# yashnaray/VQ-VAE-HMM-model

Hardware: AMD Instinct MI355X
Metric: VAE_HMM train-step sequences/sec (K=3, T=200, D=5) at 1/2/4/8 MI355X (higher is better)
Workload: dtype f32; 1 GPU; cfg2: VAE_HMM train step (compute_loss+backward+Adam); global_batch=1024, per_gpu_batch=1024, seq_len=200, K=3, input_dim=5, hidden_dim=64, hidden_dim2=32, u_dim=4, trans_hidden=128, parallelism=single, hip_graph=False, step_form=fused (Adam in the backward's tail launch), eager

## Files before the change

### vq-vae-hmm-model_amd/csrc/api.hip

```cpp
#include "vqhmm.h"

#include <math.h>
#include <stdio.h>
#include <stdlib.h>
#include <string.h>

#include <algorithm>

#include "kernels.h"


using namespace vqhmm;

namespace {

enum P {
  ENC1_W, ENC1_B, ENC2_W, ENC2_B, LOGIT_W, LOGIT_B, LOG_PRIOR, TN0_W, TN0_B, TN2_W, TN2_B,
  EMB, DEC1_W, DEC1_B, DEC2_W, DEC2_B, PAR_W, PAR_B
};

struct Carver {
  char* base;
  size_t off = 0;
  template <class T>
// ... 1247 lines not shown
      break;
    }
    case S_REDUCE: nm = p.wgroup && tail_fused_on() ? "tail" : "grad_tail"; break;
    case S_COMPOSE_BWD: nm = p.wgroup ? (tail_fused_on() ? "tail" : "adam") : "compose_bwd"; break;
    case S_LOGPRIOR: nm = p.wgroup && tail_fused_on() ? "tail" : "grad_tail"; break;
  }
  snprintf(out, len, "%s", nm);
  return VQHMM_OK;
}

int vqhmm_elbo_stage_f32(const vqhmm_dims_t* d, const float* const* w, const float* x, const float* u, int u_layout,
                         const int64_t* lengths, const int64_t* norm, int64_t B, int64_t T, float beta, void* ws,
                         size_t ws_bytes, float* grad, int stage, void* stream) {
  if (!dims_ok(d) || !w || !ws || stage < 0 || stage >= S_COUNT) return VQHMM_EINVAL;
  ElboPlan p = plan_elbo(d, B, T, ws);
  if (ws_bytes < p.bytes) return VQHMM_EWORKSPACE;
  StepCtx c{w, x, u, u_layout, lengths, norm, beta, 1, p.loss, nullptr, nullptr, grad, nullptr};
  return run_stage(p, c, stage, (hipStream_t)stream);
}

int vqhmm_elbo_pieces(const vqhmm_dims_t* d, int64_t B, int64_t T, const void* ws, const float** loss,
                      const float** pieces) {
  if (!dims_ok(d) || !ws) return VQHMM_EINVAL;
  ElboPlan p = plan_elbo(d, B, T, const_cast<void*>(ws));
  if (loss) *loss = p.loss;
  if (pieces) *pieces = p.pieces;
  return VQHMM_OK;
}

int vqhmm_elbo_status_offset(const vqhmm_dims_t* d, int64_t B, int64_t T, size_t* offset) {
  if (!dims_ok(d) || B <= 0 || T <= 0 || !offset) return VQHMM_EINVAL;
  char* const base = reinterpret_cast<char*>(4096);
  const ElboPlan p = plan_elbo(d, B, T, base);
  *offset = (size_t)(reinterpret_cast<char*>(p.sync + 2) - base);
  return VQHMM_OK;
}

int vqhmm_elbo_debug_buffers(const vqhmm_dims_t* d, int64_t B, int64_t T, const void* ws, const float** out) {
  if (!dims_ok(d) || !ws || !out) return VQHMM_EINVAL;
  ElboPlan p = plan_elbo(d, B, T, const_cast<void*>(ws));
  const float* v[16] = {p.xp, p.h1e, p.h2e, p.logits, p.q, p.g1, p.g2, p.par,
                        p.dpar, p.dg2, p.dg1, p.dqd, p.dlog, p.dh2, p.dh1, p.dqx};
  for (int i = 0; i < 16; ++i) out[i] = v[i];
  return VQHMM_OK;
}

int vqhmm_debug_prof(int which, uint64_t* out, int64_t n) {
  if (!out || n < 0 || n > 256 * 16) return VQHMM_EINVAL;
  switch (which) {
    case 0: return strip_prof_copy(out, n);
    case 1: return conv2_prof_copy(out, n);
    case 2: return head_prof_copy(out, n);
    case 3: return bwdw_prof_copy(out, n);
  }
  return VQHMM_EINVAL;
}

int vqhmm_adam_f32(float* param, const float* grad, float* exp_avg, float* exp_avg_sq, int64_t n, double lr,
                   double beta1, double beta2, double eps, int64_t* step, float grad_scale, void* stream) {
  if (n < 0 || !step || (n > 0 && (!param || !grad || !exp_avg || !exp_avg_sq))) return VQHMM_EINVAL;
  return launch_adam(param, grad, exp_avg, exp_avg_sq, n, lr, beta1, beta2, eps, step, grad_scale,
                     (hipStream_t)stream);
}

int vqhmm_clip_grad_norm_f32(float* grad, int64_t n, float pre_scale, float max_norm, float* total_norm,
                              void* stream) {
  if (n < 0 || (n > 0 && !grad) || !(max_norm > 0.f)) return VQHMM_EINVAL;
  return launch_clip_grad_norm(grad, n, pre_scale, max_norm, total_norm, (hipStream_t)stream);
}

int vqhmm_gather_chunks_f32(const float* src, const int64_t* meta, int64_t B, int64_t C, int64_t Tmax, float* out,
                            void* stream) {
  if (B < 0 || C < 0 || Tmax < 0 || C > INT32_MAX || Tmax > INT32_MAX) return VQHMM_EINVAL;
  if (B * C * Tmax > 0 && (!src || !meta || !out)) return VQHMM_EINVAL;
  return launch_gather_chunks(src, meta, B, C, Tmax, out, (hipStream_t)stream);
}

int vqhmm_infer_workspace_size(const vqhmm_dims_t* d, int64_t B, int64_t T, size_t* bytes) {
  if (!dims_ok(d) || B < 0 || T < 0 || !bytes) return VQHMM_EINVAL;
  const int64_t R = B * (T + 2);
  const int hw = ld4(d->hidden_dim > d->hidden_dim2 ? d->hidden_dim : d->hidden_dim2);
  Carver c{nullptr};
  c.take<float>(R * hw);
  c.take<float>(R * hw);
  c.take<float>(R * ld4(d->K));
  c.take<float>(R * ld4(d->input_dim > d->K ? d->input_dim : d->K));
  c.take<float>((size_t)d->hidden_dim * d->K * 3);
  *bytes = c.off + 256;
  return VQHMM_OK;
}

static int encode_impl(const vqhmm_dims_t* d, const float* const* w, const float* x, int64_t B, int64_t T,
                       float* logits_cf, float* q_cf, float* q_pcl, float* xin, float* bufA, float* bufB,
                       hipStream_t s, int32_t* regimes = nullptr) {
  const int64_t R = B * (T + 2);
  int rc;
  if ((rc = launch_to_pcl(x, d->input_dim, B, (int)T, T, 1, xin, s))) return rc;
  ConvArgs a{};
  a.R = R; a.T = (int)T;
  a.src = xin; a.Kc = d->input_dim; a.ks = 3; a.W = w[ENC1_W]; a.bias = w[ENC1_B];
  a.N = d->hidden_dim; a.act = 1; a.out = bufA;
  if ((rc = launch_conv(a, s))) return rc;
  a = ConvArgs{};
  a.R = R; a.T = (int)T;
  a.src = bufA; a.Kc = d->hidden_dim; a.ks = 3; a.W = w[ENC2_W]; a.bias = w[ENC2_B]; a.N = d->hidden_dim2;
  a.act = 1; a.out = bufB;
// ... 428 lines not shown
```

### vq-vae-hmm-model_amd/csrc/kernels.h

```cpp
#pragma once
#include "common.h"

namespace vqhmm {

struct ConvArgs {
  const float* src;
  int src_cf;
  int Kc;
  int64_t R;
  int T;
  int ks;
  const float* W;
  int w_dgrad;
  const float* Wimg;
  const float* bias;
  const float* scale;
  int N;
  int act;
  const float* aux;
  float* out;
  float* out_cf;
  const float* tW;
  const float* tb;
  int C2;
// ... 154 lines not shown
int launch_conv(const ConvArgs& a, hipStream_t s);
enum ConvKind { CONV_UNSUPPORTED, CONV_CONV2, CONV_BIG, CONV_BIG_TAIL, CONV_MM, CONV_MM_TAIL, CONV_MM_TAIL_SPLIT };
struct ConvChoice {
  int kind;
  int cfg;
  size_t lds;
};
ConvChoice conv_choice(const ConvArgs& a);
void conv_family(const ConvArgs& a, char* out, size_t n);
bool convbig_supported(const ConvArgs& a);
int launch_convbig(const ConvArgs& a, hipStream_t s);
bool conv2_supported(const ConvArgs& a);
bool conv2_fused_supported(const ConvArgs& a);
int launch_conv2_fused(const ConvArgs& a, hipStream_t s);
bool conv2_bwd_pair_supported(const ConvArgs& a, const ConvArgs& f);
int launch_conv2_bwd_pair(const ConvArgs& a, const ConvArgs& f, hipStream_t s);
struct WImgJob {
  const float* W;
  const float* E;
  int composed, H;
  int w_dgrad, N, Kc, ks;
  float* img;
};
__host__ __device__ inline int c2_nb(int N) { return N <= 16 ? 1 : N <= 32 ? 2 : 4; }
__host__ __device__ inline int c2_kcp(int Kc) { return Kc <= 16 ? 1 : Kc <= 32 ? 2 : 4; }
__host__ __device__ inline int c2_ldx(int Kc) { return 16 * c2_kcp(Kc) + 8; }
__host__ __device__ inline int64_t c2_image_floats(int N, int Kc, int ks) {
  return (int64_t)ks * 16 * c2_nb(N) * c2_ldx(Kc);
}
int launch_conv2(const ConvArgs& a, hipStream_t s);
bool strip_fwd_supported(const ConvArgs& e1, const ConvArgs& e2, const ConvArgs& d1, const ConvArgs& d2);
bool strip_head_supported(const HeadArgs& h);
int strip_fwd_grid(int64_t R);
int launch_strip_fwd(const ConvArgs& e1, const ConvArgs& e2, const ConvArgs& d1, const ConvArgs& d2, const HeadArgs* h,
                     hipStream_t s);
bool strip_bwd_supported(const ConvArgs& pd, const ConvArgs& d2, const ConvArgs& f, const ConvArgs& e2);
int launch_strip_bwd(const ConvArgs& pd, const ConvArgs& d2, const ConvArgs& f, const ConvArgs& e2, hipStream_t s);
struct StripWgradArgs {
  const float* x;
  const float* cmpW;
  float* slab[6];
  float* bslab[6];
  float* cslab;
  int D, K, H2;
  int64_t* step_inc;
  int store;
};
bool strip_bwdw_supported(const ConvArgs& pd, const ConvArgs& d2, const ConvArgs& f, const ConvArgs& e2, int D);
int strip_bwdw_own(int64_t R);
int strip_bwdw_grid(int64_t R);
int launch_strip_bwdw(const ConvArgs& pd, const ConvArgs& d2, const ConvArgs& f, const ConvArgs& e2,
                      const StripWgradArgs& w, hipStream_t s);
int strip_prof_copy(uint64_t* out, int64_t n);
int conv2_prof_copy(uint64_t* out, int64_t n);
int head_prof_copy(uint64_t* out, int64_t n);
int bwdw_prof_copy(uint64_t* out, int64_t n);
int launch_wgrad(const WgradArgs& a, hipStream_t s);
enum WgradKind { WGRAD_UNSUPPORTED, WGRAD_2, WGRAD_BIG, WGRAD_GENERIC };
int wgrad_choice(const WgradArgs& a);
const char* wgrad_family(const WgradArgs& a);
bool wgradbig_supported(const WgradArgs& a);
int64_t wgradbig_rows(int64_t R, int N, int C);
int launch_wgradbig(const WgradArgs& a, hipStream_t s);
int64_t wgrad_chunks(int64_t R, int64_t tiles);
bool wgrad2_supported(const WgradArgs& a);
int64_t wgrad2_rows(int64_t R, int N, int C, int ks);
int launch_wgrad2(const WgradArgs& a, hipStream_t s);
constexpr int MAX_WJOBS = 8;
struct WgradGroup {
  WgradArgs job[MAX_WJOBS];
  int variant[MAX_WJOBS], wn[MAX_WJOBS], wc[MAX_WJOBS];
  int64_t blk0[MAX_WJOBS + 1];
  int njobs;
  int64_t* step_inc;
};
bool wgrad2_group_supported(const WgradArgs& a);
int64_t wgrad2_group_rows(int64_t rows, int N, int C, int ks);
int launch_wgrad2_group(const WgradArgs* jobs, int n, hipStream_t s, int64_t* step_inc = nullptr);
struct StagedHeadArgs {
  int64_t B;
  int T;
  int64_t R;
  int D, K;
  const float *x, *par, *logits, *q;
  const int64_t* lengths;
  const float* log_prior;
  float* log_pi;
  float* lgA;
  float *nx, *dqc, *trw;
  float beta;
  const int64_t* norm;
  int need_grad;
  float *dpar, *dlx, *dqx;
  double* part;
  float* q0;
};
bool staged_head_supported(int K);
bool fused_head_supported(const HeadArgs& a);
enum FusedHeadKind { HEAD_NONE, HEAD_MFMA, HEAD_SCALAR };
int fused_head_kind(const HeadArgs& a);
enum StagedL1 { L1_NONE, L1_LANES16, L1_POW2_32, L1_POW2_16, L1_WIDE4, L1_WIDE, L1_LANES64 };
int staged_l1_variant(int K);
const char* staged_l1_name(int K);
int launch_staged_head(const StagedHeadArgs& a, int l2grid, hipStream_t s);

int head_grid(int64_t R);
// ... 145 lines not shown
```

### vq-vae-hmm-model_amd/csrc/strip.hip

```cpp
#include "vqhmm.h"

#include <stddef.h>
#include <stdlib.h>

#include "prof.h"
#include "strip_dev.h"

namespace vqhmm {

struct StripFwdArgs {
  int64_t R;
  int T, D, H2, K, P;
  const float* xp;
  const float *img_e1, *img_d1;
  const float *img_e2, *img_d2;
  const float *b_e1, *b_e2, *b_d1, *b_d2;
  const float *tWl, *tbl;
  const float *tWp, *tbp;
  float *h1e, *h2e, *logits, *q, *g1, *g2, *par;
  int64_t nstrip;
  int dbg;
};

namespace {

template <int NB2>
struct StripFwdLds {
  static constexpr int NW2 = 16 * NB2;
  float We2[3 * NW2 * ST_LDW];
  float Wd2[3 * 64 * ST_LDW];
  float Ee2[NW2 * 17 + 16];
  float Ed2[64 * 17 + 16];
  float Wf[2][3 * 64 * 8];
  float bf[2][64];
  float Xx[ST_XR * ST_XLD];
  float Xq[ST_XR * ST_XLD];
  float slot[8][18 * ST_LDW];
  unsigned long long hcnt[8];
};

template <int TH>
struct StripHeadW {
  static constexpr int LDW2 = TH + 4;
  float W2S[16 * LDW2];
  float W1S[TH * 8];
};
struct StripHeadLds {
  static constexpr int LDL = 20;
  float uS[ST_WIN * 8];
  float lgS[ST_WIN * LDL];
  float dlgS[ST_WIN * LDL];
  float aS[ST_WIN * 4];
  float wS[ST_WIN];
  double red[8][4];
  float q0w[8][4];
};

__device__ __forceinline__ void pk_weights(const float* Wf, int C, int lg4, int l16, float (&w)[4][4]) {
#pragma unroll
  for (int e = 0; e < 4; ++e) {
    const int k = 4 * lg4 + e;
    const bool in = k < 3 * C;
    const int tap = in ? k / C : 0, c = in ? k - tap * C : 0;
#pragma unroll
    for (int nb = 0; nb < 4; ++nb) {
      const float v = Wf[(tap * 64 + nb * 16 + l16) * 8 + c];
      w[nb][e] = in ? v : 0.f;
    }
  }
}

__device__ __forceinline__ void pk_block(const float (&w)[4][4], const float* Xw, int C, int lg4, int l16,
                                         f32x4 (&acc)[4]) {
  float b[4];
#pragma unroll
  for (int e = 0; e < 4; ++e) {
    const int k = 4 * lg4 + e;
    const bool in = k < 3 * C;
    const int tap = in ? k / C : 0, c = in ? k - tap * C : 0;
    const float v = Xw[(l16 + tap) * ST_XLD + c];
    b[e] = in ? v : 0.f;
  }
#pragma unroll
  for (int nb = 0; nb < 4; ++nb) {
    acc[nb] = f32x4{0.f, 0.f, 0.f, 0.f};
#pragma unroll
    for (int e = 0; e < 4; ++e) acc[nb] = mfma16x16x4(w[nb][e], b[e], acc[nb]);
  }
}

__device__ __forceinline__ void front_epi(f32x4 (&acc)[4], const f32x4 (&bias)[4], int64_t r0, int64_t R, int T,
                                          int lg4, int l16, int slo, int shi, float* out, float* xs,
                                          bool nostore, int only = -1, float* xlo = nullptr,
                                          float* xhi = nullptr) {
  const int64_t r = r0 + l16;
  const bool valid = row_valid(r, R, T);
  const bool st = l16 >= slo && l16 < shi && r < R && !nostore;
#pragma unroll
  for (int nb = 0; nb < 4; ++nb) {
    f32x4 y;
#pragma unroll
    for (int v = 0; v < 4; ++v) {
      const float yy = relu_f(acc[nb][v] * 1.0f + bias[nb][v]);
      y[v] = valid ? yy : 0.f;
    }
    acc[nb] = y;
    if (st) *reinterpret_cast<f32x4*>(out + r * 64 + nb * 16 + 4 * lg4) = y;
    if (only < 0 || l16 == only) *reinterpret_cast<f32x4*>(xs + l16 * ST_LDW + nb * 16 + 4 * lg4) = y;
    if (xlo && l16 == 0) *reinterpret_cast<f32x4*>(xlo + nb * 16 + 4 * lg4) = y;
    if (xhi && l16 == 15) *reinterpret_cast<f32x4*>(xhi + nb * 16 + 4 * lg4) = y;
  }
}

template <int NB>
struct TailConsts {
  f32x4 bias[NB], tw[NB], tb;
  __device__ __forceinline__ void load(const float* Es, int lg4, int l16) {
    constexpr int NW = 16 * NB;
#pragma unroll
    for (int nb = 0; nb < NB; ++nb) {
      const float4 b4 = *reinterpret_cast<const float4*>(Es + nb * 16 + 4 * lg4);
      const float4 t4 = *reinterpret_cast<const float4*>(Es + NW + l16 * NW + nb * 16 + 4 * lg4);
      bias[nb] = f32x4{b4.x, b4.y, b4.z, b4.w};
      tw[nb] = f32x4{t4.x, t4.y, t4.z, t4.w};
    }
    const float4 t4 = *reinterpret_cast<const float4*>(Es + 17 * NW + 4 * lg4);
    tb = f32x4{t4.x, t4.y, t4.z, t4.w};
  }
};

template <int NB, bool SM>
__device__ __forceinline__ void tail_epi(f32x4 (&acc)[NB], const TailConsts<NB>& k, int64_t r0, int64_t R, int T,
                                         int lg4, int l16, int slo, int shi, int N, float* out, int C2, float* t_out,
                                         float* q_out, float* xq, bool nostore) {
  const int64_t r = r0 + l16;
  const bool valid = row_valid(r, R, T);
  const bool st = l16 >= slo && l16 < shi && r < R && !nostore;
  const int ldn = ld4(N), ldt = ld4(C2);
#pragma unroll
  for (int nb = 0; nb < NB; ++nb) {
    f32x4 y;
#pragma unroll
    for (int v = 0; v < 4; ++v) {
      const float yy = relu_f(acc[nb][v] * 1.0f + k.bias[nb][v]);
      y[v] = valid ? yy : 0.f;
    }
    acc[nb] = y;
    const int n0 = nb * 16 + 4 * lg4;
    if (st && n0 < ldn) *reinterpret_cast<f32x4*>(out + r * ldn + n0) = y;
  }
  f32x4 z = k.tb;
#pragma unroll
  for (int nb = 0; nb < NB; ++nb)
#pragma unroll
    for (int v = 0; v < 4; ++v) z = mfma16x16x4(k.tw[nb][v], acc[nb][v], z);
  const int c0 = 4 * lg4;
#pragma unroll
  for (int v = 0; v < 4; ++v) z[v] = valid ? z[v] : 0.f;
  if (st && c0 < ldt) *reinterpret_cast<f32x4*>(t_out + r * ldt + c0) = z;
  if constexpr (SM) {
    float m = -__builtin_inff();
#pragma unroll
    for (int v = 0; v < 4; ++v)
      if (c0 + v < C2) m = fmaxf(m, z[v]);
    m = fmaxf(m, xor16(m));
    m = fmaxf(m, xor32(m));
    float e[4], s = 0.f;
#pragma unroll
    for (int v = 0; v < 4; ++v) {
      e[v] = (c0 + v < C2) ? __expf(z[v] - m) : 0.f;
      s += e[v];
    }
    s += xor16(s);
    s += xor32(s);
    f32x4 qv;
#pragma unroll
    for (int v = 0; v < 4; ++v) qv[v] = valid ? e[v] / s : 0.f;
    if (st && c0 < ldt) *reinterpret_cast<f32x4*>(q_out + r * ldt + c0) = qv;
    if (c0 == 0) {
      *reinterpret_cast<f32x4*>(xq + l16 * ST_XLD) = qv;
      *reinterpret_cast<f32x4*>(xq + l16 * ST_XLD + 4) = z;
    }
  }
}

template <int NW>
__device__ __forceinline__ const float* es_src(const float* bias, int N, const float* tW, const float* tb, int C2, int i,
                                               bool& ok) {
  const bool in_b = i < NW, in_w = !in_b && i < 17 * NW;
  const int j = in_w ? i - NW : 0, c2w = j / NW, n = j - c2w * NW, c2b = (!in_b && !in_w) ? i - 17 * NW : 0;
// ... 43 lines not shown

  auto load_x = [&](int64_t s0) {
    const int row = tid >> 1, h = 4 * (tid & 1);
    int64_t r = s0 - 2 + row;
    r = r < 0 ? 0 : (r >= R ? R - 1 : r);
    return *reinterpret_cast<const float4*>(a.xp + r * ldx + (h < ldx ? h : 0));
  };
  auto store_x = [&](int64_t s0, float4 v) {
    if (tid < 2 * ST_XR) {
      const int row = tid >> 1, h = 4 * (tid & 1);
      const int64_t r = s0 - 2 + row;
      const bool ok = r >= 0 && r < R && h < ldx;
      *reinterpret_cast<float4*>(sh.Xx + row * ST_XLD + h) = ok ? v : make_float4(0.f, 0.f, 0.f, 0.f);
    }
  };

  constexpr int HKP = 4, HB = HTH > 0 ? HTH / 16 : 1, HLDW2 = HTH + 4, HNW = HTH > 0 ? 16 * HLDW2 + HTH * 8 : 1;
  constexpr int HNJ = (HNW + 511) / 512;
  const int prow = tid >> 2, si = tid & 3;
  float hwv[HNJ];
  if constexpr (HTH > 0) {
    const int KK = h.K * h.K;
#pragma unroll
    for (int j = 0; j < HNJ; ++j) {
      const int i = tid + 512 * j;
      float v = 0.f;
      if (i < 16 * HLDW2) {
        const int ij = i / HLDW2, hh = i - ij * HLDW2;
        v = (ij < KK && hh < HTH) ? h.W2[ij * HTH + hh] : 0.f;
      } else if (i < HNW) {
        const int k = i - 16 * HLDW2, hh = k >> 3, c = k & 7;
        v = c < h.U ? h.W1[hh * h.U + c] : (c == h.U ? h.b1[hh] : 0.f);
      }
      hwv[j] = v;
    }
    if (!h.norm && !h.cnt_in) {
      unsigned long long c = 0;
      for (int64_t b = tid; b < h.B; b += 512) {
        const int64_t L = h.lengths[b];
        c += (unsigned long long)(L <= 0 ? 0 : (L < T ? L : T));
      }
#pragma unroll
      for (int o = 32; o >= 1; o >>= 1) c += __shfl_xor(c, o);
      if (lane == 0) sh.hcnt[wave] = c;
    }
  }
  stamp<PROF>(0);
  if constexpr (PROF > 0) { if (threadIdx.x == 0 && blockIdx.x < 256) g_prof[blockIdx.x * 16 + 13] = __builtin_amdgcn_s_memtime(); }
  for (int j = wave; wave < 4 && j < 12; j += 4) {
    const int g = j * 64 + lane, img = g / 384, i = g - img * 384, row = i >> 1, h = 4 * (i & 1);
    dma16((img ? a.img_d1 : a.img_e1) + row * ST_LDF + h, &sh.Wf[0][0] + j * 256);
  }
  int64_t s = blockIdx.x;
  float4 px = load_x(s * ST_OWN - ST_HALO);
  constexpr int NE = NW2 * 17 + 16, ND = 64 * 17 + 16, NC = NE + ND + 128;
  constexpr int NCJ = (NC + 511) / 512;
  float cv[NCJ];
  bool cvok[NCJ];
#pragma unroll
  for (int j = 0; j < NCJ; ++j) {
    const int i = tid + 512 * j;
    bool oke, okd;
    const float* pe = es_src<NW2>(a.b_e2, a.H2, a.tWl, a.tbl, a.K, i < NE ? i : 0, oke);
    const float* pd = es_src<64>(a.b_d2, 64, a.tWp, a.tbp, a.P, (i >= NE && i < NE + ND) ? i - NE : 0, okd);
    const int ib = (i >= NE + ND && i < NC) ? i - NE - ND : 0;
    const bool inE = i < NE, inD = !inE && i < NE + ND, inB = !inE && !inD && i < NC;
    const bool ok = inE ? oke : inD ? okd : inB;
    const float* p = inE ? pe : inD ? pd : (ib < 64 ? a.b_e1 : a.b_d1) + (ib & 63);
    cv[j] = *(ok ? p : a.b_e1);
    cvok[j] = ok;
  }
#pragma unroll
  for (int j = 0; j < NCJ; ++j) cv[j] = cvok[j] ? cv[j] : 0.f;
  {
    constexpr int N1 = 3 * NW2 * ST_LDW / 4, N2 = 3 * 64 * ST_LDW / 4;
    constexpr int C1 = (N1 + 63) / 64, C2 = (N2 + 63) / 64;
    constexpr int NJ = (C1 + C2 + 7) / 8;
#pragma unroll
    for (int jj = 0; jj < NJ; ++jj) {
      const int c = min(wave + 8 * jj, C1 + C2 - 1);
      const bool first = c < C1;
      const int cc = first ? c : c - C1;
      const int i = cc * 64 + lane;
      if (i < (first ? N1 : N2)) dma16((first ? a.img_e2 : a.img_d2) + 4 * i, (first ? sh.We2 : sh.Wd2) + cc * 256);
    }
  }
  static_assert(offsetof(S, Ed2) == offsetof(S, Ee2) + NE * 4, "constant blocks must be contiguous");
#pragma unroll
  for (int j = 0; j < NCJ; ++j) {
    const int i = tid + 512 * j;
    if (i < NE + ND) sh.Ee2[i] = cv[j];
    else if (i < NC) sh.bf[0][i - NE - ND] = cv[j];
  }
  if (tid < 4 * ST_XLD) sh.Xq[(tid < 2 * ST_XLD ? 0 : (ST_XR - 4) * ST_XLD) + tid] = 0.f;
  store_x(s * ST_OWN - ST_HALO, px);
  lds_barrier();
  stamp<PROF>(1);
  float wE[4][4], wD[4][4];
  pk_weights(sh.Wf[0], a.D, lg4, l16, wE);
  pk_weights(sh.Wf[1], a.K, lg4, l16, wD);
  f32x4 bE[4], bD[4];
#pragma unroll
  for (int nb = 0; nb < 4; ++nb) {
    const float4 e4 = *reinterpret_cast<const float4*>(sh.bf[0] + nb * 16 + 4 * lg4);
    const float4 d4 = *reinterpret_cast<const float4*>(sh.bf[1] + nb * 16 + 4 * lg4);
    bE[nb] = f32x4{e4.x, e4.y, e4.z, e4.w};
    bD[nb] = f32x4{d4.x, d4.y, d4.z, d4.w};
  }
  TailConsts<NB2> kE;
  TailConsts<4> kD;
  if constexpr (HTH == 0) {
    kE.load(sh.Ee2, lg4, l16);
    kD.load(sh.Ed2, lg4, l16);
  }
  static_assert(HTH == 0 || (offsetof(S, Xx) == offsetof(S, bf) + 2 * 64 * 4 &&
                             sizeof(StripHeadW<HTH>) <= offsetof(S, Xx) - offsetof(S, Wf) &&
                             sizeof(StripHeadLds) <= sizeof(float) * 8 * 18 * ST_LDW),
                "the head's LDS fits the regions it reuses");
  float lp_i = 0.f, inv_n = 1.f, cpri = 0.f, cent = 0.f;
  const bool hgrad = h.need_grad != 0;
  if constexpr (HTH > 0) {
    unsigned long long cnt;
    if (h.norm) cnt = (unsigned long long)h.norm[0];
    else if (h.cnt_in) cnt = (unsigned long long)*h.cnt_in;
    else cnt = ((((((sh.hcnt[0] + sh.hcnt[1]) + sh.hcnt[2]) + sh.hcnt[3]) + sh.hcnt[4]) + sh.hcnt[5]) + sh.hcnt[6]) + sh.hcnt[7];
    inv_n = 1.0f / fmaxf((float)(cnt * (unsigned long long)h.D), 1.0f);
    const float Bn = loss_norm_batch(h.norm, h.B);
    cpri = -h.beta / Bn;
    cent = h.beta / Bn;
    float m = -__builtin_inff();
    for (int k = 0; k < h.K; ++k) m = fmaxf(m, h.log_prior[k]);
    float se = 0.f;
    for (int k = 0; k < h.K; ++k) se += __expf(h.log_prior[k] - m);
    if (si < h.K) lp_i = h.log_prior[si] - (m + __logf(se));
  }
  float s_rec = 0.f, s_ent = 0.f, s_tr = 0.f, s_init = 0.f, q0acc = 0.f, db2acc = 0.f;
  f32x4 gW2 = f32x4{0.f, 0.f, 0.f, 0.f}, gW1 = gW2;

  const int mlo = ST_HALO - 16 * wave, mhi = ST_HALO + ST_OWN - 16 * wave;
  const int slo = max(0, mlo), shi = min(16, mhi);
  const bool nost = a.dbg & 1;
  int it = 0;
  for (; s < a.nstrip; s += gridDim.x) {
    const int64_t s0 = s * ST_OWN - ST_HALO;
    const int64_t rb = s0 + 16 * wave;
    {
      const int64_t nx = s + gridDim.x;
      px = load_x((nx < a.nstrip ? nx : s) * ST_OWN - ST_HALO);
    }
    {
      f32x4 acc[4];
      pk_block(wE, sh.Xx + (16 * wave + 1) * ST_XLD, a.D, lg4, l16, acc);
      front_epi(acc, bE, rb, R, T, lg4, l16, slo, shi, a.h1e, slot + ST_LDW, nost, -1,
                wave > 0 ? sh.slot[wave - 1] + 17 * ST_LDW : nullptr, wave < 7 ? sh.slot[wave + 1] : nullptr);
      if (wave == 5 || wave == 6) {
        const bool lo = wave == 5;
        f32x4 acc2[4];
        pk_block(wE, sh.Xx + (lo ? 0 : 16 * 7 + 2) * ST_XLD, a.D, lg4, l16, acc2);
        front_epi(acc2, bE, lo ? s0 - 1 : s0 + 16 * 7 + 1, R, T, lg4, l16, 0, 0, a.h1e,
                  lo ? sh.slot[0] : sh.slot[7] + 2 * ST_LDW, true, lo ? 0 : 15);
      }
    }
    if (it == 0) asm volatile("s_waitcnt vmcnt(0)" ::: "memory");
    lds_barrier();
    {
      f32x4 acc[NB2][1];
#pragma unroll
      for (int nb = 0; nb < NB2; ++nb) acc[nb][0] = f32x4{0.f, 0.f, 0.f, 0.f};
      c2_mfma_tile<NB2, 1, 4, 3, ST_LDW, NW2>(sh.We2, slot, lg4, l16, acc, true);
      f32x4 y[NB2];
#pragma unroll
      for (int nb = 0; nb < NB2; ++nb) y[nb] = acc[nb][0];
      if constexpr (HTH > 0) kE.load(sh.Ee2, lg4, l16);
      tail_epi<NB2, true>(y, kE, rb, R, T, lg4, l16, slo, shi, a.H2, a.h2e, a.K, a.logits, a.q,
                          sh.Xq + (16 * wave + 2) * ST_XLD, nost);
    }
    lds_barrier();
    if (it == 0) stamp<PROF>(2);
    if constexpr (HTH > 0) {
      if (it == 0) {
        float* hw = &sh.Wf[0][0];
#pragma unroll
        for (int j = 0; j < HNJ; ++j)
          if (tid + 512 * j < HNW) hw[tid + 512 * j] = hwv[j];
      }
    }
    {
      f32x4 acc[4];
      pk_block(wD, sh.Xq + (16 * wave + 1) * ST_XLD, a.K, lg4, l16, acc);
      if constexpr (PROF > 0) {
        if (it == 0) {
          asm volatile("s_nop 0" : : "v"(acc[3][3]));
          stamp<PROF>(10);
        }
      }
      front_epi(acc, bD, rb, R, T, lg4, l16, slo, shi, a.g1, slot + ST_LDW, nost, -1,
                wave > 0 ? sh.slot[wave - 1] + 17 * ST_LDW : nullptr, wave < 7 ? sh.slot[wave + 1] : nullptr);
      if (it == 0) stamp<PROF>(11);
    }
    lds_barrier();
    if (it == 0) stamp<PROF>(4);
    {
      f32x4 acc[4][1];
#pragma unroll
      for (int nb = 0; nb < 4; ++nb) acc[nb][0] = f32x4{0.f, 0.f, 0.f, 0.f};
      c2_mfma_tile<4, 1, 4, 3, ST_LDW, 64>(sh.Wd2, slot, lg4, l16, acc, true);
      f32x4 y[4];
#pragma unroll
      for (int nb = 0; nb < 4; ++nb) y[nb] = acc[nb][0];
      if constexpr (PROF > 0) {
        if (it == 0) {
          asm volatile("s_nop 0" : : "v"(y[3][3]));
          stamp<PROF>(5);
        }
      }
      if constexpr (HTH > 0) kD.load(sh.Ed2, lg4, l16);
      tail_epi<4, false>(y, kD, rb, R, T, lg4, l16, slo, shi, 64, a.g2, a.P, a.par, nullptr, nullptr, nost);
    }
    if (it == 0) stamp<PROF>(6);
    {
      const int64_t nx = s + gridDim.x;
      store_x((nx < a.nstrip ? nx : s) * ST_OWN - ST_HALO, px);
    }
    if constexpr (HTH > 0) __syncthreads();
    else lds_barrier();
    if (it == 0) stamp<PROF>(3);
    if constexpr (HTH > 0) {
      StripHeadLds& hs = *reinterpret_cast<StripHeadLds*>(&sh.slot[0][0]);
      const StripHeadW<HTH>& hw = *reinterpret_cast<const StripHeadW<HTH>*>(&sh.Wf[0][0]);
      constexpr int LDL = StripHeadLds::LDL;
      const int K = h.K, U = h.U, D = h.D, KK = K * K;
      const int ldp = ld4(2 * D), ldxh = ld4(D), ldu = ld4(U);
      const int64_t r = s0 + ST_HALO + prow;
      const unsigned Tp = (unsigned)T + 2u;
      const unsigned rcl = (unsigned)(r < R ? r : R - 1);
      const int b = (int)(rcl / Tp);
      const int t = (int)(rcl - (unsigned)b * Tp) - 1;
      const bool valid = r < R && prow <= ST_OWN && t >= 0 && t < T;
      const bool own = prow < ST_OWN && r < R;
      const int64_t L = h.lengths[b];
      const bool m = valid && t < L;
      const float wgt = (valid && t >= 1 && t < L) ? 1.f : 0.f;
      const float* qrow = sh.Xq + (ST_HALO + prow + 2) * ST_XLD;
      float qv[HKP];
#pragma unroll
      for (int k = 0; k < HKP; ++k) qv[k] = (valid && k < K) ? qrow[k] : 0.f;
      const float qp = (valid && t >= 1 && si < K) ? qrow[si - ST_XLD] : 0.f;
      float qi = 0.f;
#pragma unroll
      for (int k = 0; k < HKP; ++k) qi = si == k ? qv[k] : qi;
      float mu[2], lv[2], xv[2];
#pragma unroll
      for (int k = 0; k < 2; ++k) {
        const int c = min(si + HKP * k, D - 1);
        mu[k] = h.par[(int64_t)rcl * ldp + c];
        lv[k] = h.par[(int64_t)rcl * ldp + D + c];
        xv[k] = h.x[(int64_t)rcl * ldxh + c];
      }
      const float uu = h.u[(int64_t)rcl * ldu + min(si, ldu - 1)];
#pragma unroll
      for (int c = si; c < 8; c += HKP) hs.uS[prow * 8 + c] = c < U ? (valid ? uu : 0.f) : (c == U ? 1.f : 0.f);
      for (int i = tid; i < ST_WIN * LDL; i += 512)
        if (i % LDL >= KK) hs.dlgS[i] = 0.f;
      lds_barrier();
      {
        f32x4 lg;
#pragma unroll
        for (int v = 0; v < 4; ++v) {
          const int ij = 4 * lg4 + v;
          lg[v] = ij < KK ? h.b2[ij] : 0.f;
        }
        const float ub = hs.uS[(wave * 16 + l16) * 8 + lg4];
#pragma unroll 2
        for (int hb = 0; hb < HB; ++hb) {
          const float w1a = lg4 < U ? hw.W1S[(hb * 16 + l16) * 8 + lg4] : 0.f;
          f32x4 bb;
#pragma unroll
          for (int v = 0; v < 4; ++v) bb[v] = hw.W1S[(hb * 16 + 4 * lg4 + v) * 8 + U];
// ... 330 lines not shown
      for (int nb = 0; nb < 4; ++nb) y[nb] = acc[nb][0];
      mask_epi(y, m2, 1.0f, rb, R, T, lg4, l16, slo, shi, a.dh1, nullptr, 0);
    }
    ++it;
  }
  if constexpr (PROF > 0) {
    __syncthreads();
    stamp<PROF>(7);
    if (threadIdx.x == 0 && blockIdx.x < 256) g_prof[blockIdx.x * 16 + 8] = (unsigned long long)it;
  }
}

bool strip_bwd_supported(const ConvArgs& pd, const ConvArgs& d2, const ConvArgs& f, const ConvArgs& e2) {
  return pd.R > 0 && pd.R < (1ll << 31) && pd.ks == 1 && pd.act == 2 && pd.Wimg && pd.aux && pd.out && pd.N == 64 &&
         pd.Kc >= 1 && pd.Kc <= 16 && !pd.src_cf && !pd.bias &&
         d2.src == pd.out && d2.ks == 3 && d2.act == 2 && d2.Wimg && d2.aux && d2.out && d2.Kc == 64 && d2.N == 64 &&
         !d2.bias && !d2.scale &&
         f.src == d2.out && f.act == 3 && f.ks == 3 && f.Wimg && f.Kc == 64 && f.N >= 1 && f.N <= 4 && f.lb_dh &&
         f.lb_C > 16 && f.lb_C <= 32 && ld4(f.lb_C) == 32 && !f.bias && !f.out_cf &&
         e2.src == f.lb_dh && e2.ks == 3 && e2.act == 2 && e2.Wimg && e2.aux && e2.out && e2.Kc == f.lb_C &&
         e2.N == 64 && !e2.bias && !e2.scale && !e2.tW && !e2.out_cf;
}

int launch_strip_bwd(const ConvArgs& pd, const ConvArgs& d2, const ConvArgs& f, const ConvArgs& e2, hipStream_t s) {
  if (!strip_bwd_supported(pd, d2, f, e2)) return VQHMM_EUNSUPPORTED;
  StripBwdArgs a{};
  a.R = pd.R; a.T = pd.T; a.ldp = ld4(pd.Kc);
  a.dpar = pd.src; a.g2 = pd.aux; a.g1 = d2.aux; a.h1e = e2.aux;
  a.img_pd = pd.Wimg; a.img_d2 = d2.Wimg; a.img_c1 = f.Wimg; a.img_e2 = e2.Wimg;
  a.gscale = pd.scale;
  a.dg2 = pd.out; a.dg1 = d2.out; a.dh1 = e2.out;
  a.nstrip = cdiv(pd.R, ST_OWN);
  const unsigned grid = (unsigned)(a.nstrip < 256 ? a.nstrip : 256);
  if (prof_on()) strip_bwd_kernel<1><<<grid, 512, sizeof(StripBwdLds), s>>>(a, f);
  else strip_bwd_kernel<0><<<grid, 512, sizeof(StripBwdLds), s>>>(a, f);
  VQHMM_LAUNCH_CHECK();
  return VQHMM_OK;
}

static StripFwdArgs strip_fwd_args(const ConvArgs& e1, const ConvArgs& e2, const ConvArgs& d1, const ConvArgs& d2) {
  StripFwdArgs a{};
  a.R = e1.R; a.T = e1.T; a.D = e1.Kc; a.H2 = e2.N; a.K = e2.C2; a.P = d2.C2;
  a.xp = e1.src;
  a.img_e1 = e1.Wimg; a.img_d1 = d1.Wimg; a.img_e2 = e2.Wimg; a.img_d2 = d2.Wimg;
  a.b_e1 = e1.bias; a.b_e2 = e2.bias; a.b_d1 = d1.bias; a.b_d2 = d2.bias;
  a.tWl = e2.tW; a.tbl = e2.tb; a.tWp = d2.tW; a.tbp = d2.tb;
  a.h1e = e1.out; a.h2e = e2.out; a.logits = e2.t_out; a.q = e2.q_out; a.g1 = d1.out; a.g2 = d2.out; a.par = d2.t_out;
  a.nstrip = cdiv(e1.R, ST_OWN);
  static const int dbg = [] {
    const char* e = VQHMM_PROF_ENV("VQHMM_STRIP_DBG");
    return e ? atoi(e) : 0;
  }();
  a.dbg = dbg;
  return a;
}

bool strip_fwd_supported(const ConvArgs& e1, const ConvArgs& e2, const ConvArgs& d1, const ConvArgs& d2) {
  auto relu3 = [](const ConvArgs& a) { return a.ks == 3 && a.act == 1 && !a.src_cf && a.Wimg && a.out && !a.out_cf; };
  return relu3(e1) && relu3(e2) && relu3(d1) && relu3(d2) && e1.R > 0 && e1.R < (1ll << 31) &&
         e1.Kc >= 1 && 3 * e1.Kc <= 16 && e1.N == 64 &&
         e2.src == e1.out && e2.Kc == 64 && e2.N >= 1 && e2.N <= 32 &&
         e2.C2 >= 1 && e2.C2 <= 4 && e2.t_out && e2.q_out && !e2.q_cf && !e2.reg_out && !e2.t_cf0 &&
         d1.src == e2.q_out && d1.Kc == e2.C2 && 3 * d1.Kc <= 16 && d1.N == 64 &&
         d2.src == d1.out && d2.Kc == 64 && d2.N == 64 && d2.C2 >= 1 && d2.C2 <= 16 && d2.t_out && !d2.t_cf0 &&
         !d2.q_out && !d2.q_cf && !d2.reg_out;
}

int strip_prof_copy(uint64_t* out, int64_t n) { return prof_copy(out, n); }

bool strip_head_supported(const HeadArgs& h) {
  return h.K >= 1 && h.K <= 4 && h.U >= 1 && h.U <= 4 && (h.TH == 64 || h.TH == 128) && h.D >= 1 && h.D <= 8 &&
         h.R < (1ll << 31);
}

int strip_fwd_grid(int64_t R) {
  const int64_t n = cdiv(R, ST_OWN);
  return (int)(n < 256 ? (n > 0 ? n : 1) : 256);
}

int launch_strip_fwd(const ConvArgs& e1, const ConvArgs& e2, const ConvArgs& d1, const ConvArgs& d2, const HeadArgs* h,
                     hipStream_t s) {
  if (!strip_fwd_supported(e1, e2, d1, d2)) return VQHMM_EUNSUPPORTED;
  if (h && (!strip_head_supported(*h) || h->K != e2.C2 || h->R != e1.R || h->D != e1.Kc)) return VQHMM_EUNSUPPORTED;
  const StripFwdArgs a = strip_fwd_args(e1, e2, d1, d2);
  const unsigned grid = (unsigned)strip_fwd_grid(e1.R);
  const HeadArgs hv = h ? *h : HeadArgs{};
  const int hth = h ? h->TH : 0;
#define VQHMM_SF(NB2, P, HT) strip_fwd_kernel<NB2, P, HT><<<grid, 512, sizeof(StripFwdLds<NB2>), s>>>(a, hv)
#define VQHMM_SF_H(NB2, P) \
  if (hth == 128) VQHMM_SF(NB2, P, 128); else if (hth == 64) VQHMM_SF(NB2, P, 64); else VQHMM_SF(NB2, P, 0);
  const bool prof = prof_on() != 0;
  if (c2_nb(e2.N) == 1) {
    if (prof) { VQHMM_SF_H(1, 1) } else { VQHMM_SF_H(1, 0) }
  } else {
    if (prof) { VQHMM_SF_H(2, 1) } else { VQHMM_SF_H(2, 0) }
  }
#undef VQHMM_SF_H
#undef VQHMM_SF
  VQHMM_LAUNCH_CHECK();
  return VQHMM_OK;
}

}
```

Measured before the change: 2.654 million sequences/s.

## Restructure strip forward front layers with precomputed LDS pointers and paired MFMA

Precomputes per-lane LDS source pointers, validity and store masks once outside the strip loop instead of recomputing them each iteration. Waves 5 and 6 now interleave MFMAs for their main and extra halo blocks in one pass. The next strip's x prefetch moves to the top of the loop. Adds opt-in per-phase timing points and a debug copy path, which are compiled out when PROF is off.

```diff
diff --git a/vq-vae-hmm-model_amd/csrc/api.hip b/vq-vae-hmm-model_amd/csrc/api.hip
--- a/vq-vae-hmm-model_amd/csrc/api.hip
+++ b/vq-vae-hmm-model_amd/csrc/api.hip
@@ -1323,6 +1323,7 @@
     case 1: return conv2_prof_copy(out, n);
     case 2: return head_prof_copy(out, n);
     case 3: return bwdw_prof_copy(out, n);
+    case 4: return strip_fwd_points_copy(out, n);
   }
   return VQHMM_EINVAL;
 }
diff --git a/vq-vae-hmm-model_amd/csrc/kernels.h b/vq-vae-hmm-model_amd/csrc/kernels.h
--- a/vq-vae-hmm-model_amd/csrc/kernels.h
+++ b/vq-vae-hmm-model_amd/csrc/kernels.h
@@ -230,6 +230,7 @@
 int launch_strip_bwdw(const ConvArgs& pd, const ConvArgs& d2, const ConvArgs& f, const ConvArgs& e2,
                       const StripWgradArgs& w, hipStream_t s);
 int strip_prof_copy(uint64_t* out, int64_t n);
+int strip_fwd_points_copy(uint64_t* out, int64_t n);
 int conv2_prof_copy(uint64_t* out, int64_t n);
 int head_prof_copy(uint64_t* out, int64_t n);
 int bwdw_prof_copy(uint64_t* out, int64_t n);
diff --git a/vq-vae-hmm-model_amd/csrc/strip.hip b/vq-vae-hmm-model_amd/csrc/strip.hip
--- a/vq-vae-hmm-model_amd/csrc/strip.hip
+++ b/vq-vae-hmm-model_amd/csrc/strip.hip
@@ -20,9 +20,49 @@
   float *h1e, *h2e, *logits, *q, *g1, *g2, *par;
   int64_t nstrip;
   int dbg;
+  int prof_it;
 };
 
 namespace {
+
+enum {
+  FWD_TOP, FWD_E1_READS, FWD_E1_MFMA, FWD_E1_EPI, FWD_B1, FWD_E2_LOOP, FWD_STORE_X, FWD_E2_TAIL, FWD_B2,
+  FWD_D1_READS, FWD_D1_MFMA, FWD_D1_EPI, FWD_B3, FWD_D2_LOOP, FWD_D2_TAIL, FWD_B4, FWD_NPT
+};
+static_assert(FWD_NPT == 16, "one g_prof row");
+__device__ unsigned long long g_prof_fwd[256 * 16];
+
+template <int PROF>
+struct FwdClock {
+  unsigned t[PROF > 0 ? FWD_NPT : 1];
+  __device__ __forceinline__ void clear() {
+    if constexpr (PROF > 0) {
+#pragma unroll
+      for (int k = 0; k < FWD_NPT; ++k) t[k] = 0;
+    }
+  }
+  __device__ __forceinline__ void at(int k) {
+    if constexpr (PROF > 0) {
+      __builtin_amdgcn_sched_barrier(0);
+      t[k] = (unsigned)__builtin_amdgcn_s_memrealtime();
+      __builtin_amdgcn_sched_barrier(0);
+    }
+  }
+  __device__ __forceinline__ void after(int k, float v) {
+    if constexpr (PROF > 0) {
+      asm volatile("s_nop 0" : : "v"(v));
+      at(k);
+    }
+  }
+  __device__ __forceinline__ void keep(bool on) {
+    if constexpr (PROF > 0) {
+      if (on && threadIdx.x == 0 && blockIdx.x < 256) {
+#pragma unroll
+        for (int k = 0; k < FWD_NPT; ++k) g_prof_fwd[blockIdx.x * 16 + k] = t[k];
+      }
+    }
+  }
+};
 
 template <int NB2>
 struct StripFwdLds {
@@ -70,17 +110,40 @@
   }
 }
 
-__device__ __forceinline__ void pk_block(const float (&w)[4][4], const float* Xw, int C, int lg4, int l16,
-                                         f32x4 (&acc)[4]) {
+typedef __attribute__((address_space(3))) float* ldsp;
+__device__ __forceinline__ ldsp to_lds(float* p) { return (ldsp)p; }
+
+__device__ __forceinline__ bool row_valid_flat(int64_t r, int64_t R, int T) {
+  const bool inr = r >= 0 && r < R;
+  const unsigned Tp = (unsigned)T + 2u, m = (unsigned)(inr ? r : 0) % Tp;
+  return inr && m >= 1u && m <= (unsigned)T;
+}
+
+struct PkSrc {
+  ldsp p[4];
+  bool in[4];
+  __device__ __forceinline__ void init(float* Xw, int C, int lg4, int l16) {
+#pragma unroll
+    for (int e = 0; e < 4; ++e) {
+      const int k = 4 * lg4 + e;
+      in[e] = k < 3 * C;
+      const int tap = in[e] ? k / C : 0, c = in[e] ? k - tap * C : 0;
+      p[e] = to_lds(Xw) + ((l16 + tap) * ST_XLD + c);
+      asm volatile("" : "+v"(p[e]));
+    }
+  }
+  __device__ __forceinline__ void read(int d, float (&raw)[4]) const {
+#pragma unroll
+    for (int e = 0; e < 4; ++e) raw[e] = p[e][d];
+    __builtin_amdgcn_sched_barrier(0);
+  }
+};
+
+__device__ __forceinline__ void pk_mma(const float (&w)[4][4], const float (&raw)[4], const bool (&in)[4],
+                                       f32x4 (&acc)[4]) {
   float b[4];
 #pragma unroll
-  for (int e = 0; e < 4; ++e) {
-    const int k = 4 * lg4 + e;
-    const bool in = k < 3 * C;
-    const int tap = in ? k / C : 0, c = in ? k - tap * C : 0;
-    const float v = Xw[(l16 + tap) * ST_XLD + c];
-    b[e] = in ? v : 0.f;
-  }
+  for (int e = 0; e < 4; ++e) b[e] = in[e] ? raw[e] : 0.f;
 #pragma unroll
   for (int nb = 0; nb < 4; ++nb) {
     acc[nb] = f32x4{0.f, 0.f, 0.f, 0.f};
@@ -88,14 +151,29 @@
     for (int e = 0; e < 4; ++e) acc[nb] = mfma16x16x4(w[nb][e], b[e], acc[nb]);
   }
 }
-
-__device__ __forceinline__ void front_epi(f32x4 (&acc)[4], const f32x4 (&bias)[4], int64_t r0, int64_t R, int T,
-                                          int lg4, int l16, int slo, int shi, float* out, float* xs,
-                                          bool nostore, int only = -1, float* xlo = nullptr,
-                                          float* xhi = nullptr) {
-  const int64_t r = r0 + l16;
-  const bool valid = row_valid(r, R, T);
-  const bool st = l16 >= slo && l16 < shi && r < R && !nostore;
+__device__ __forceinline__ void pk_mma2(const float (&w)[4][4], const float (&rawA)[4], const float (&rawB)[4],
+                                        const bool (&in)[4], f32x4 (&accA)[4], f32x4 (&accB)[4]) {
+  float bA[4], bB[4];
+#pragma unroll
+  for (int e = 0; e < 4; ++e) {
+    bA[e] = in[e] ? rawA[e] : 0.f;
+    bB[e] = in[e] ? rawB[e] : 0.f;
+  }
+#pragma unroll
+  for (int nb = 0; nb < 4; ++nb) {
+    accA[nb] = f32x4{0.f, 0.f, 0.f, 0.f};
+    accB[nb] = f32x4{0.f, 0.f, 0.f, 0.f};
+  }
+#pragma unroll
+  for (int e = 0; e < 4; ++e)
+#pragma unroll
+    for (int nb = 0; nb < 4; ++nb) {
+      accA[nb] = mfma16x16x4(w[nb][e], bA[e], accA[nb]);
+      accB[nb] = mfma16x16x4(w[nb][e], bB[e], accB[nb]);
+    }
+}
+
+__device__ __forceinline__ void front_act(f32x4 (&acc)[4], const f32x4 (&bias)[4], bool valid) {
 #pragma unroll
   for (int nb = 0; nb < 4; ++nb) {
     f32x4 y;
@@ -105,10 +183,30 @@
       y[v] = valid ? yy : 0.f;
     }
     acc[nb] = y;
-    if (st) *reinterpret_cast<f32x4*>(out + r * 64 + nb * 16 + 4 * lg4) = y;
-    if (only < 0 || l16 == only) *reinterpret_cast<f32x4*>(xs + l16 * ST_LDW + nb * 16 + 4 * lg4) = y;
-    if (xlo && l16 == 0) *reinterpret_cast<f32x4*>(xlo + nb * 16 + 4 * lg4) = y;
-    if (xhi && l16 == 15) *reinterpret_cast<f32x4*>(xhi + nb * 16 + 4 * lg4) = y;
+  }
+}
+
+__device__ __forceinline__ void front_epi(f32x4 (&acc)[4], const f32x4 (&bias)[4], bool valid, bool st, float* gout,
+                                          ldsp xrow, bool halo, ldsp xhalo) {
+  front_act(acc, bias, valid);
+  if (st) {
+#pragma unroll
+    for (int nb = 0; nb < 4; ++nb) *reinterpret_cast<f32x4*>(gout + nb * 16) = acc[nb];
+  }
+#pragma unroll
+  for (int nb = 0; nb < 4; ++nb) *reinterpret_cast<__attribute__((address_space(3))) f32x4*>(xrow + nb * 16) = acc[nb];
+  if (halo) {
+#pragma unroll
+    for (int nb = 0; nb < 4; ++nb) *reinterpret_cast<__attribute__((address_space(3))) f32x4*>(xhalo + nb * 16) = acc[nb];
+  }
+}
+
+__device__ __forceinline__ void front_epi_row(f32x4 (&acc)[4], const f32x4 (&bias)[4], bool valid, bool mine,
+                                              ldsp xrow) {
+  front_act(acc, bias, valid);
+  if (mine) {
+#pragma unroll
+    for (int nb = 0; nb < 4; ++nb) *reinterpret_cast<__attribute__((address_space(3))) f32x4*>(xrow + nb * 16) = acc[nb];
   }
 }
 
@@ -130,12 +228,9 @@
 };
 
 template <int NB, bool SM>
-__device__ __forceinline__ void tail_epi(f32x4 (&acc)[NB], const TailConsts<NB>& k, int64_t r0, int64_t R, int T,
-                                         int lg4, int l16, int slo, int shi, int N, float* out, int C2, float* t_out,
-                                         float* q_out, float* xq, bool nostore) {
-  const int64_t r = r0 + l16;
-  const bool valid = row_valid(r, R, T);
-  const bool st = l16 >= slo && l16 < shi && r < R && !nostore;
+__device__ __forceinline__ void tail_epi(f32x4 (&acc)[NB], const TailConsts<NB>& k, int64_t r, bool valid, bool st,
+                                         int lg4, int l16, int N, float* out, int C2, float* t_out, float* q_out,
+                                         float* xq) {
   const int ldn = ld4(N), ldt = ld4(C2);
 #pragma unroll
   for (int nb = 0; nb < NB; ++nb) {
@@ -285,7 +380,7 @@
     dma16((img ? a.img_d1 : a.img_e1) + row * ST_LDF + h, &sh.Wf[0][0] + j * 256);
   }
   int64_t s = blockIdx.x;
-  float4 px = load_x(s * ST_OWN - ST_HALO);
+  const float4 px0 = load_x(s * ST_OWN - ST_HALO);
   constexpr int NE = NW2 * 17 + 16, ND = 64 * 17 + 16, NC = NE + ND + 128;
   constexpr int NCJ = (NC + 511) / 512;
   float cv[NCJ];
@@ -326,7 +421,7 @@
     else if (i < NC) sh.bf[0][i - NE - ND] = cv[j];
   }
   if (tid < 4 * ST_XLD) sh.Xq[(tid < 2 * ST_XLD ? 0 : (ST_XR - 4) * ST_XLD) + tid] = 0.f;
-  store_x(s * ST_OWN - ST_HALO, px);
+  store_x(s * ST_OWN - ST_HALO, px0);
   lds_barrier();
   stamp<PROF>(1);
   float wE[4][4], wD[4][4];
@@ -372,30 +467,53 @@
 
   const int mlo = ST_HALO - 16 * wave, mhi = ST_HALO + ST_OWN - 16 * wave;
   const int slo = max(0, mlo), shi = min(16, mhi);
-  const bool nost = a.dbg & 1;
+  const bool stl = l16 >= slo && l16 < shi && !(a.dbg & 1);
+  PkSrc srcE, srcD;
+  srcE.init(sh.Xx + (16 * wave + 1) * ST_XLD, a.D, lg4, l16);
+  srcD.init(sh.Xq + (16 * wave + 1) * ST_XLD, a.K, lg4, l16);
+  const ldsp xrow = to_lds(slot + (1 + l16) * ST_LDW + 4 * lg4);
+  const bool halo = (l16 == 0 && wave > 0) || (l16 == 15 && wave < 7);
+  const ldsp xhalo =
+      to_lds((l16 == 0 ? sh.slot[max(wave - 1, 0)] + 17 * ST_LDW : sh.slot[min(wave + 1, 7)]) + 4 * lg4);
+  const int wu = __builtin_amdgcn_readfirstlane(wave);
+  const bool extra = wu == 5 || wu == 6, xlo = wu == 5;
+  const int xd = ((xlo ? 0 : 16 * 7 + 2) - (16 * wu + 1)) * ST_XLD;
+  const bool xmine = l16 == (xlo ? 0 : 15);
+  const ldsp xouter = to_lds((xlo ? sh.slot[0] : sh.slot[7] + 17 * ST_LDW) + 4 * lg4);
   int it = 0;
+  [[maybe_unused]] FwdClock<PROF> clk;
+  clk.clear();
   for (; s < a.nstrip; s += gridDim.x) {
     const int64_t s0 = s * ST_OWN - ST_HALO;
     const int64_t rb = s0 + 16 * wave;
+    const int64_t snx = (s + gridDim.x < a.nstrip ? s + gridDim.x : s) * ST_OWN - ST_HALO;
+    clk.at(FWD_TOP);
+    const float4 px = load_x(snx);
+    const int64_t r = rb + l16;
+    const bool valid = row_valid_flat(r, R, T), st = stl && r < R;
     {
-      const int64_t nx = s + gridDim.x;
-      px = load_x((nx < a.nstrip ? nx : s) * ST_OWN - ST_HALO);
-    }
-    {
+      float xa[4];
       f32x4 acc[4];
-      pk_block(wE, sh.Xx + (16 * wave + 1) * ST_XLD, a.D, lg4, l16, acc);
-      front_epi(acc, bE, rb, R, T, lg4, l16, slo, shi, a.h1e, slot + ST_LDW, nost, -1,
-                wave > 0 ? sh.slot[wave - 1] + 17 * ST_LDW : nullptr, wave < 7 ? sh.slot[wave + 1] : nullptr);
-      if (wave == 5 || wave == 6) {
-        const bool lo = wave == 5;
+      srcE.read(0, xa);
+      if (extra) {
+        float xb[4];
         f32x4 acc2[4];
-        pk_block(wE, sh.Xx + (lo ? 0 : 16 * 7 + 2) * ST_XLD, a.D, lg4, l16, acc2);
-        front_epi(acc2, bE, lo ? s0 - 1 : s0 + 16 * 7 + 1, R, T, lg4, l16, 0, 0, a.h1e,
-                  lo ? sh.slot[0] : sh.slot[7] + 2 * ST_LDW, true, lo ? 0 : 15);
-      }
-    }
+        srcE.read(xd, xb);
+        const bool valid2 = row_valid_flat(xlo ? s0 - 1 : s0 + ST_WIN, R, T);
+        pk_mma2(wE, xa, xb, srcE.in, acc, acc2);
+        front_epi(acc, bE, valid, st, a.h1e + r * 64 + 4 * lg4, xrow, halo, xhalo);
+        front_epi_row(acc2, bE, valid2, xmine, xouter);
+      } else {
+        clk.at(FWD_E1_READS);
+        pk_mma(wE, xa, srcE.in, acc);
+        clk.after(FWD_E1_MFMA, acc[3][3]);
+        front_epi(acc, bE, valid, st, a.h1e + r * 64 + 4 * lg4, xrow, halo, xhalo);
+      }
+    }
+    clk.at(FWD_E1_EPI);
     if (it == 0) asm volatile("s_waitcnt vmcnt(0)" ::: "memory");
     lds_barrier();
+    clk.at(FWD_B1);
     {
       f32x4 acc[NB2][1];
 #pragma unroll
@@ -404,11 +522,14 @@
       f32x4 y[NB2];
 #pragma unroll
       for (int nb = 0; nb < NB2; ++nb) y[nb] = acc[nb][0];
+      clk.after(FWD_E2_LOOP, y[NB2 - 1][3]);
       if constexpr (HTH > 0) kE.load(sh.Ee2, lg4, l16);
-      tail_epi<NB2, true>(y, kE, rb, R, T, lg4, l16, slo, shi, a.H2, a.h2e, a.K, a.logits, a.q,
-                          sh.Xq + (16 * wave + 2) * ST_XLD, nost);
-    }
+      tail_epi<NB2, true>(y, kE, r, valid, st, lg4, l16, a.H2, a.h2e, a.K, a.logits, a.q,
+                          sh.Xq + (16 * wave + 2) * ST_XLD);
+    }
+    clk.at(FWD_E2_TAIL);
     lds_barrier();
+    clk.at(FWD_B2);
     if (it == 0) stamp<PROF>(2);
     if constexpr (HTH > 0) {
       if (it == 0) {
@@ -419,19 +540,24 @@
       }
     }
     {
+      float xa[4];
       f32x4 acc[4];
-      pk_block(wD, sh.Xq + (16 * wave + 1) * ST_XLD, a.K, lg4, l16, acc);
+      srcD.read(0, xa);
+      clk.at(FWD_D1_READS);
+      pk_mma(wD, xa, srcD.in, acc);
+      clk.after(FWD_D1_MFMA, acc[3][3]);
       if constexpr (PROF > 0) {
         if (it == 0) {
           asm volatile("s_nop 0" : : "v"(acc[3][3]));
           stamp<PROF>(10);
         }
       }
-      front_epi(acc, bD, rb, R, T, lg4, l16, slo, shi, a.g1, slot + ST_LDW, nost, -1,
-                wave > 0 ? sh.slot[wave - 1] + 17 * ST_LDW : nullptr, wave < 7 ? sh.slot[wave + 1] : nullptr);
+      front_epi(acc, bD, valid, st, a.g1 + r * 64 + 4 * lg4, xrow, halo, xhalo);
       if (it == 0) stamp<PROF>(11);
     }
+    clk.at(FWD_D1_EPI);
     lds_barrier();
+    clk.at(FWD_B3);
     if (it == 0) stamp<PROF>(4);
     {
       f32x4 acc[4][1];
@@ -441,6 +567,7 @@
       f32x4 y[4];
 #pragma unroll
       for (int nb = 0; nb < 4; ++nb) y[nb] = acc[nb][0];
+      clk.after(FWD_D2_LOOP, y[3][3]);
       if constexpr (PROF > 0) {
         if (it == 0) {
           asm volatile("s_nop 0" : : "v"(y[3][3]));
@@ -448,15 +575,16 @@
         }
       }
       if constexpr (HTH > 0) kD.load(sh.Ed2, lg4, l16);
-      tail_epi<4, false>(y, kD, rb, R, T, lg4, l16, slo, shi, 64, a.g2, a.P, a.par, nullptr, nullptr, nost);
-    }
+      tail_epi<4, false>(y, kD, r, valid, st, lg4, l16, 64, a.g2, a.P, a.par, nullptr, nullptr);
+    }
+    clk.at(FWD_D2_TAIL);
     if (it == 0) stamp<PROF>(6);
-    {
-      const int64_t nx = s + gridDim.x;
-      store_x((nx < a.nstrip ? nx : s) * ST_OWN - ST_HALO, px);
-    }
+    store_x(snx, px);
+    clk.at(FWD_STORE_X);
     if constexpr (HTH > 0) __syncthreads();
     else lds_barrier();
+    clk.at(FWD_B4);
+    clk.keep(it == a.prof_it);
     if (it == 0) stamp<PROF>(3);
     if constexpr (HTH > 0) {
       StripHeadLds& hs = *reinterpret_cast<StripHeadLds*>(&sh.slot[0][0]);
@@ -893,6 +1021,8 @@
     return e ? atoi(e) : 0;
   }();
   a.dbg = dbg;
+  static const int pit = prof_env("VQHMM_STRIP_PROF_IT");
+  a.prof_it = pit;
   return a;
 }
 
@@ -908,6 +1038,9 @@
 }
 
 int strip_prof_copy(uint64_t* out, int64_t n) { return prof_copy(out, n); }
+int strip_fwd_points_copy(uint64_t* out, int64_t n) {
+  return hipMemcpyFromSymbol(out, HIP_SYMBOL(g_prof_fwd), (size_t)n * 8, 0, hipMemcpyDeviceToHost) == hipSuccess ? 0 : -2;
+}
 
 bool strip_head_supported(const HeadArgs& h) {
   return h.K >= 1 && h.K <= 4 && h.U >= 1 && h.U <= 4 && (h.TH == 64 || h.TH == 128) && h.D >= 1 && h.D <= 8 &&
```

After: 2.672 million sequences/s (median of 6 runs). Within noise of the previous version (+0.7%).
